# haesungpyun/seoul_tourism_recommendation_NGCF

Measured on AMD Instinct MI355X. Metric: NGCF 3-layer forward: propagated edges/sec + achieved HBM GB/s, d=128, higher is better.
Workload: dtype f32

## Files before the change

seoul_tourism_recommendation_ngcf_amd/csrc/common.h:

```cpp
#ifndef NGCF_COMMON_H
#define NGCF_COMMON_H

#include <hip/hip_runtime.h>

#include <algorithm>
#include <cstdarg>
#include <cstdint>
#include <cstdio>
#include <cstdlib>
#include <cstring>
#include <numeric>
#include <thread>
#include <vector>

#include "../../include/ngcf_hip.h"

inline thread_local char g_err[512] = "";

inline int fail(int code, const char *fmt, ...)
{
    va_list ap;
    va_start(ap, fmt);
    vsnprintf(g_err, sizeof(g_err), fmt, ap);
    va_end(ap);
    return code;
}

#define HIP_TRY(expr)                                                                          \
    do {                                                                                       \
        hipError_t e_ = (expr);                                                                \
        if (e_ != hipSuccess)                                                                  \
            return fail(NGCF_ERR_HIP, "%s failed: %s (%s:%d)", #expr, hipGetErrorString(e_),   \
                        __FILE__, __LINE__);                                                   \
    } while (0)

#define LAUNCH_CHECK()                                                                         \
    do {                                                                                       \
        hipError_t e_ = hipGetLastError();                                                     \
        if (e_ != hipSuccess)                                                                  \
            return fail(NGCF_ERR_HIP, "kernel launch failed: %s (%s:%d)", hipGetErrorString(e_), \
                        __FILE__, __LINE__);                                                   \
    } while (0)


struct NgcfOptions {
    int no_fork = 0;
    int no_slicing = 0;
    int no_ldstab = 0;
    int no_panel_split = 0;
    int no_tail_table = 0;
    int no_pad_product = 0;
    int64_t fork_min = 200000000;
    int dense_direct = 1;
    int dense_resident = 4;
    int dense_resident_min_rows = 106496;
    int dense_small_tiles = 1;
    int dense_tall = 1;
    int t_rows_bitmap = 1;
    int bwd_input_resident = 1;
    int select_no_lds = 0;
    int slice_max_mb = 48;
    int swept_lpe = 16;
    int swept_cut = 4;
    int swept_no_moments = 0;
    int swept_order_rows = 0;
    int swept_debug = 0;
    int swept_window_kb = 0;
    int swept_spin = 500;
    int swept_lead = -2;
    int swept_sync_every = 1;
    int swept_prio_kb = 256;
    int swept_prio_graded = 1;
};
extern NgcfOptions g_opts;
const NgcfOptions &ngcf_opts();


constexpr int kMaxDevices = 64;
inline int current_device_slot()
{
    int dev = 0;
    if (hipGetDevice(&dev) != hipSuccess || dev < 0) dev = 0;
    return dev % kMaxDevices;
}

template <auto kernel> static hipError_t allow_full_lds(int bytes = 160 * 1024)
{
    static bool set[kMaxDevices] = {};
    const int dev_i = current_device_slot();
    if (set[dev_i]) return hipSuccess;
    const hipError_t e = hipFuncSetAttribute(reinterpret_cast<const void *>(kernel), hipFuncAttributeMaxDynamicSharedMemorySize, bytes);
    set[dev_i] = e == hipSuccess;
    return e;
}

inline int64_t align_up(int64_t x, int64_t a) { return (x + a - 1) / a * a; }
inline bool aligned16(const void *p) { return (reinterpret_cast<uintptr_t>(p) & 15) == 0; }


inline int grid_for(int64_t n, int block)

{
    int64_t g = (n + block - 1) / block;
    if (g < 1) g = 1;
    if (g > 256 * 16) g = 256 * 16;
    return (int)g;
}



struct ngcf_csr {
    int64_t n_rows = 0, n_cols = 0, nnz = 0;
    int64_t max_row_len = 0;
    int64_t *rowptr = nullptr;
    int32_t *colidx = nullptr;
    float *vals = nullptr;
    bool owns = false;
    int64_t cap = 0, pos_len = 0;
    int32_t *pos = nullptr;
    int32_t *scan_blk = nullptr;
    bool borrows_plan = false;
    const struct ngcf_csr *filter_src = nullptr;
    int32_t seg_len = 0;
    int64_t n_seg = 0, n_heavy = 0;
    int32_t *seg_row = nullptr;
    int64_t *seg_begin = nullptr;
    int32_t *heavy_row = nullptr;
    int64_t *heavy_seg_ptr = nullptr;
    struct RowGroup {
        int64_t begin, end;
        bool sliceable;
        int32_t col_lo, col_hi;
        bool lds_table = false;
    };
    std::vector<RowGroup> groups;
    int mode = 0;
    struct SegSet {
        int64_t n_seg = 0, n_heavy = 0;
        int32_t *seg_row = nullptr;
        int64_t *seg_begin = nullptr;
        int32_t *heavy_row = nullptr;
        int64_t *heavy_seg_ptr = nullptr;
    };
    struct Swept {
        struct Part {
            int64_t row_lo = 0, row_hi = 0;
            int waves = 0, rows_per_wave = 0;
            int lpe = 16;
            int32_t n_rowpass = 0, n_win = 0, win_cols = 0, col_lo = 0, col_hi = 0;
            int64_t n_slots = 0, n_partial = 0, n_heavy = 0, partial_base = 0;
            int64_t *tptr = nullptr;
            int32_t *e_pack = nullptr;
            float *e_val = nullptr;
            int32_t *dst = nullptr;
            int32_t *prow = nullptr;
            int32_t *heavy_row = nullptr;
            int64_t *heavy_seg_ptr = nullptr;
        };
        std::vector<Part> parts;
        std::vector<char> group_swept;
        SegSet out;
        int64_t n_partial = 0;
        uint32_t *barrier = nullptr;
        mutable hipStream_t barrier_owner[4] = {nullptr, nullptr, nullptr, nullptr};
        mutable int barrier_used = 0;
        int built_mode = 0;
        int lpe = 16;
    } swept;
};


static const int32_t kLdsTableRows = 512;
static const int32_t kDefaultSegLen = 2048;
static inline int32_t default_seg_len(int64_t nnz)
{
    int32_t s = 64;
    while (s < kDefaultSegLen && (int64_t)s * 4096 < nnz) s *= 2;
    return s;
}

void free_swept(ngcf_csr *c);
int build_swept_plan(ngcf_csr *c, hipStream_t stream);
bool swept_usable(const ngcf_csr *c, int64_t ldE, int d);
void prof_mark(hipStream_t stream, int which);

__host__ __device__ inline uint64_t fmix64(uint64_t x)
{
    x ^= x >> 33;
    x *= 0xff51afd7ed558ccdULL;
    x ^= x >> 33;
    x *= 0xc4ceb9fe1a85ec53ULL;
    x ^= x >> 33;
    return x;
}
__device__ inline uint32_t mix32(uint64_t x) { return (uint32_t)fmix64(x); }

__device__ __forceinline__ uint32_t msg_drop_thr(float drop_p)
{
    return drop_p > 0.f ? (uint32_t)((double)drop_p * 4294967296.0) : 0u;
}
__device__ __forceinline__ float msg_drop(float v, uint64_t seed, int64_t row, int col, uint32_t thr, float keep_scale)
{
    const uint32_t h = mix32(seed ^ ((uint64_t)row * 0x9E3779B97F4A7C15ULL + (uint64_t)col));
    return h < thr ? 0.f : v * keep_scale;
}

constexpr uint64_t kSeedPtrTag = 0xD5EDull;
__device__ inline uint64_t resolve_seed(uint64_t s)
{
    if ((s >> 48) == kSeedPtrTag) s = *reinterpret_cast<const uint64_t *>(s & 0xFFFFFFFFFFFFull);
    const uint32_t lo = __builtin_amdgcn_readfirstlane((uint32_t)s), hi = __builtin_amdgcn_readfirstlane((uint32_t)(s >> 32));
    return ((uint64_t)hi << 32) | lo;
}

struct EdgeDrop {
    int n;
    uint32_t thr;
    uint64_t seed[4];
    int transposed;
};

struct EdgeDropR {
    int n;
    uint32_t thr;
    uint64_t s0, s1, s2, s3;
// ... 116 lines not shown
```

seoul_tourism_recommendation_ngcf_amd/csrc/csr.hip:

```cpp
#include "common.h"

extern "C" const char *ngcf_last_error(void) { return g_err; }
extern "C" const char *ngcf_target_arch(void) { return "gfx950"; }
extern "C" int ngcf_version(void) { return NGCF_ABI_VERSION; }

NgcfOptions g_opts;

namespace {
struct OptField {
    const char *name;
    int NgcfOptions::*i;
    int64_t NgcfOptions::*l;
};
const OptField kOptFields[] = {
    {"no_fork", &NgcfOptions::no_fork, nullptr},
    {"no_slicing", &NgcfOptions::no_slicing, nullptr},
    {"no_ldstab", &NgcfOptions::no_ldstab, nullptr},
    {"no_panel_split", &NgcfOptions::no_panel_split, nullptr},
    {"no_tail_table", &NgcfOptions::no_tail_table, nullptr},
    {"no_pad_product", &NgcfOptions::no_pad_product, nullptr},
    {"fork_min", nullptr, &NgcfOptions::fork_min},
    {"dense_direct", &NgcfOptions::dense_direct, nullptr},
    {"dense_resident", &NgcfOptions::dense_resident, nullptr},
    {"dense_resident_min_rows", &NgcfOptions::dense_resident_min_rows, nullptr},
    {"dense_small_tiles", &NgcfOptions::dense_small_tiles, nullptr},
    {"dense_tall", &NgcfOptions::dense_tall, nullptr},
    {"bwd_input_resident", &NgcfOptions::bwd_input_resident, nullptr},
    {"t_rows_bitmap", &NgcfOptions::t_rows_bitmap, nullptr},
    {"select_no_lds", &NgcfOptions::select_no_lds, nullptr},
    {"slice_max_mb", &NgcfOptions::slice_max_mb, nullptr},
    {"swept_lpe", &NgcfOptions::swept_lpe, nullptr},
    {"swept_cut", &NgcfOptions::swept_cut, nullptr},
    {"swept_no_moments", &NgcfOptions::swept_no_moments, nullptr},
    {"swept_order_rows", &NgcfOptions::swept_order_rows, nullptr},
    {"swept_debug", &NgcfOptions::swept_debug, nullptr},
    {"swept_window_kb", &NgcfOptions::swept_window_kb, nullptr},
    {"swept_spin", &NgcfOptions::swept_spin, nullptr},
    {"swept_lead", &NgcfOptions::swept_lead, nullptr},
    {"swept_sync_every", &NgcfOptions::swept_sync_every, nullptr},
    {"swept_prio_kb", &NgcfOptions::swept_prio_kb, nullptr},
    {"swept_prio_graded", &NgcfOptions::swept_prio_graded, nullptr},
};
bool g_opts_read = false;
}

extern "C" int ngcf_options_from_env(void)
{
    NgcfOptions o;
    for (const OptField &f : kOptFields) {
        char var[64] = "NGCF_";
        size_t n = strlen(var);
        for (const char *p = f.name; *p && n + 1 < sizeof(var); ++p) var[n++] = (char)((*p >= 'a' && *p <= 'z') ? *p - 32 : *p);
        var[n] = 0;
        const char *e = getenv(var);
        if (!e) continue;
        const long long v = *e ? atoll(e) : 1;
        if (f.i) o.*(f.i) = (int)(*e && (*e == '-' || (*e >= '0' && *e <= '9')) ? v : 1);
        else o.*(f.l) = v;
    }
    if (const char *e = getenv("NGCF_SWEPT_ORDER")) o.swept_order_rows = !strcmp(e, "rows");
    g_opts = o;
    g_opts_read = true;
    return NGCF_OK;
}

const NgcfOptions &ngcf_opts()
{
    if (!g_opts_read) ngcf_options_from_env();
    return g_opts;
}

extern "C" int ngcf_set_option(const char *name, int64_t value)
{
    if (!name) return fail(NGCF_ERR_ARG, "ngcf_set_option: null name");
    (void)ngcf_opts();
    for (const OptField &f : kOptFields)
        if (!strcmp(f.name, name)) {
            if (f.i) g_opts.*(f.i) = (int)value;
            else g_opts.*(f.l) = value;
            return NGCF_OK;
        }
    return fail(NGCF_ERR_ARG, "ngcf_set_option: unknown option '%s'", name);
}


static void free_plan(ngcf_csr *c)
{
    if (c->borrows_plan) {
        c->seg_row = nullptr;
        c->heavy_row = nullptr;
        c->heavy_seg_ptr = nullptr;
        c->borrows_plan = false;
    }
    if (c->seg_row) (void)hipFree(c->seg_row);
    if (c->seg_begin) (void)hipFree(c->seg_begin);
    if (c->heavy_row) (void)hipFree(c->heavy_row);
    if (c->heavy_seg_ptr) (void)hipFree(c->heavy_seg_ptr);
    c->seg_row = nullptr;
    c->seg_begin = nullptr;
    c->heavy_row = nullptr;
    c->heavy_seg_ptr = nullptr;
    c->n_seg = c->n_heavy = 0;
}

extern "C" void ngcf_csr_free(ngcf_csr_t *c)
{
    if (!c) return;
    free_plan(c);
    free_swept(c);
    if (c->owns) {
        if (c->rowptr) (void)hipFree(c->rowptr);
        if (c->colidx) (void)hipFree(c->colidx);
        if (c->vals) (void)hipFree(c->vals);
    }
    if (c->pos) (void)hipFree(c->pos);
    if (c->scan_blk) (void)hipFree(c->scan_blk);
    delete c;
}

extern "C" int64_t ngcf_csr_nnz(const ngcf_csr_t *c) { return c ? c->nnz : -1; }
extern "C" int64_t ngcf_csr_n_rows(const ngcf_csr_t *c) { return c ? c->n_rows : -1; }
extern "C" int64_t ngcf_csr_n_cols(const ngcf_csr_t *c) { return c ? c->n_cols : -1; }
extern "C" int64_t ngcf_csr_n_segments(const ngcf_csr_t *c) { return c ? c->n_seg : -1; }
extern "C" int64_t ngcf_csr_max_row_len(const ngcf_csr_t *c) { return c ? c->max_row_len : -1; }
extern "C" int64_t ngcf_csr_swept_rows(const ngcf_csr_t *c)
{
    if (!c) return -1;
    int64_t n = 0;
    for (const auto &p : c->swept.parts) n += p.row_hi - p.row_lo;
    return n;
}
extern "C" const int64_t *ngcf_csr_rowptr(const ngcf_csr_t *c) { return c ? c->rowptr : nullptr; }
extern "C" const int32_t *ngcf_csr_colidx(const ngcf_csr_t *c) { return c ? c->colidx : nullptr; }
extern "C" const float *ngcf_csr_vals(const ngcf_csr_t *c) { return c ? c->vals : nullptr; }

__global__ void coo_check_kernel(const int64_t *__restrict__ rows, const int64_t *__restrict__ cols,
                                 int64_t nnz, int64_t n_rows, int64_t n_cols, int32_t *flags)
{
    int64_t i = (int64_t)blockIdx.x * blockDim.x + threadIdx.x;
    const int64_t stride = (int64_t)gridDim.x * blockDim.x;
    bool unsorted = false, bad = false;
    for (; i < nnz; i += stride) {
        const int64_t r = rows[i], c = cols[i];
        bad |= (r < 0) | (r >= n_rows) | (c < 0) | (c >= n_cols);
        if (i + 1 < nnz) unsorted |= rows[i + 1] < r;
    }
    if (unsorted) atomicOr(&flags[0], 1);
    if (bad) atomicOr(&flags[1], 1);
}

__global__ void coo_rowptr_kernel(const int64_t *__restrict__ rows, int64_t nnz, int64_t n_rows,
                                  int64_t *__restrict__ rowptr)
{
    const int64_t r = (int64_t)blockIdx.x * blockDim.x + threadIdx.x;
    if (r > n_rows) return;
    int64_t lo = 0, hi = nnz;
    while (lo < hi) {
        const int64_t mid = (lo + hi) >> 1;
        if (rows[mid] < r)
            lo = mid + 1;
        else
            hi = mid;
    }
    rowptr[r] = lo;
}

__global__ void coo_copy_kernel(const int64_t *__restrict__ cols, const float *__restrict__ vals, int64_t nnz,
                                int32_t *__restrict__ colidx, float *__restrict__ out_vals)
{
    int64_t i = (int64_t)blockIdx.x * blockDim.x + threadIdx.x;
    const int64_t stride = (int64_t)gridDim.x * blockDim.x;
    for (; i < nnz; i += stride) {
        colidx[i] = (int32_t)cols[i];
        out_vals[i] = vals[i];
    }
}


__global__ void row_colrange_kernel(const int64_t *__restrict__ rowptr, const int32_t *__restrict__ colidx,
                                    int64_t n_rows, int group_rows, int32_t *__restrict__ blk_min, int32_t *__restrict__ blk_max)
{
    const int64_t row = (int64_t)blockIdx.x * blockDim.x + threadIdx.x;
    if (row >= n_rows) return;
    int32_t lo = INT32_MAX, hi = -1;
    for (int64_t e = rowptr[row]; e < rowptr[row + 1]; ++e) {
        const int32_t c = colidx[e];
        lo = c < lo ? c : lo;
        hi = c > hi ? c : hi;
    }
    if (hi >= 0) {
        atomicMin(&blk_min[row / group_rows], lo);
        atomicMax(&blk_max[row / group_rows], hi);
    }
}
// ... 451 lines not shown
```

seoul_tourism_recommendation_ngcf_amd/csrc/spmm_swept.hip:

```cpp
#include "spmm_device.h"

namespace {
constexpr int kLdsBytes = 36 * 16 * 256;
constexpr int kSweptWGs = 256;
constexpr int kRing = 8;
constexpr int kRowBits = 24;
constexpr int kColMask = (1 << kRowBits) - 1;

template <typename F>
void parallel_for(int64_t n, F &&fn, int64_t min_parallel = 64)
{
    unsigned nt = std::thread::hardware_concurrency();
    if (nt > 16) nt = 16;
    if (nt < 1) nt = 1;
    if ((int64_t)nt > n) nt = (unsigned)std::max<int64_t>(n, 1);
    if (n < min_parallel || nt == 1) {
        fn(0, n);
        return;
    }
    std::vector<std::thread> th;
    const int64_t chunk = (n + nt - 1) / nt;
    for (unsigned t = 0; t < nt; ++t) {
        const int64_t lo = t * chunk, hi = std::min<int64_t>(n, lo + chunk);
        if (lo >= hi) break;
        th.emplace_back([&fn, lo, hi]() { fn(lo, hi); });
    }
    for (auto &t : th) t.join();
}

void free_part(ngcf_csr::Swept::Part &p)
{
    if (p.tptr) (void)hipFree(p.tptr);
    if (p.e_pack) (void)hipFree(p.e_pack);
    if (p.e_val) (void)hipFree(p.e_val);
    if (p.dst) (void)hipFree(p.dst);
    if (p.prow) (void)hipFree(p.prow);
    if (p.heavy_row) (void)hipFree(p.heavy_row);
    if (p.heavy_seg_ptr) (void)hipFree(p.heavy_seg_ptr);
    p = ngcf_csr::Swept::Part();
}

void free_segset(ngcf_csr::SegSet &s)
{
    if (s.seg_row) (void)hipFree(s.seg_row);
    if (s.seg_begin) (void)hipFree(s.seg_begin);
    if (s.heavy_row) (void)hipFree(s.heavy_row);
    if (s.heavy_seg_ptr) (void)hipFree(s.heavy_seg_ptr);
    s = ngcf_csr::SegSet();
}

template <typename T>
int upload(T **dptr, const std::vector<T> &h, hipStream_t stream)
{
    HIP_TRY(hipMalloc(dptr, sizeof(T) * std::max<size_t>(h.size(), 1)));
    if (!h.empty()) HIP_TRY(hipMemcpyAsync(*dptr, h.data(), sizeof(T) * h.size(), hipMemcpyHostToDevice, stream));
    return NGCF_OK;
}

struct Piece {
    int64_t row;
    int64_t begin, end, count;
    int32_t off, step;
    int64_t src;
};

int build_part(const ngcf_csr *c, const ngcf_csr::RowGroup &grp, bool force, hipStream_t stream, ngcf_csr::Swept::Part &part, int LPE)
{
    const int kSW = LPE * 4, kEPR = 64 / LPE, kLdsRows = kLdsBytes / (kSW * 4);
    const int64_t row_lo = grp.begin, row_hi = grp.end, n = row_hi - row_lo;
    const int32_t col_lo = grp.col_lo, col_hi = grp.col_hi;
    if (n <= 0 || col_hi < col_lo) return NGCF_OK;
    if (col_hi > kColMask) return NGCF_OK;
    std::vector<int64_t> rp((size_t)n + 1);
    HIP_TRY(hipMemcpyAsync(rp.data(), c->rowptr + row_lo, sizeof(int64_t) * rp.size(), hipMemcpyDeviceToHost, stream));
    HIP_TRY(hipStreamSynchronize(stream));
    const int64_t e0 = rp[0], nnz = rp[(size_t)n] - e0;
    if (nnz <= 0) return NGCF_OK;
    if (!force && nnz < ((int64_t)1 << 22)) return NGCF_OK;
    const int64_t cap = (int64_t)kSweptWGs * kLdsRows;
    const int waves = 16;
    const int RW = kLdsRows / waves;
    const int64_t n_wave_slots = (int64_t)kSweptWGs * waves;
    if (!force) {
        const double span = (double)col_hi - col_lo + 1;
        const double reuse = (double)nnz / span * std::min(1.0, (double)(cap / 8) / (double)n);
        if (reuse < 3.0 || span * kSW * 4 < (double)(8 << 20)) return NGCF_OK;
    }
    std::vector<int32_t> col((size_t)nnz);
    std::vector<float> val((size_t)nnz);
    HIP_TRY(hipMemcpyAsync(col.data(), c->colidx + e0, sizeof(int32_t) * (size_t)nnz, hipMemcpyDeviceToHost, stream));
    HIP_TRY(hipMemcpyAsync(val.data(), c->vals + e0, sizeof(float) * (size_t)nnz, hipMemcpyDeviceToHost, stream));
    HIP_TRY(hipStreamSynchronize(stream));
    for (auto &x : rp) x -= e0;
    int64_t n_rowpass = std::max<int64_t>(1, (n + cap - 1) / cap), n_tasks = 0, T = 0, n_partial = 0;
    std::vector<Piece> pieces;
    std::vector<int32_t> heavy_row;
    std::vector<int64_t> heavy_ptr;
    for (;; ++n_rowpass) {
        n_tasks = n_rowpass * n_wave_slots;
        T = std::max<int64_t>(64, (nnz + n_tasks - 1) / n_tasks);
        const int64_t Tp = std::max<int64_t>(64, T / std::max(2, ngcf_opts().swept_cut));
        pieces.clear();
        heavy_row.clear();
        heavy_ptr.assign(1, 0);
        n_partial = 0;
        for (int64_t r = 0; r < n; ++r) {
            const int64_t b = rp[(size_t)r], e = rp[(size_t)r + 1], len = e - b;
            if (len <= Tp) {
                pieces.push_back({r, b, e, len, 0, 1, r});
            } else {
                const int64_t k = (len + Tp - 1) / Tp;
                heavy_row.push_back((int32_t)(row_lo + r));
                for (int64_t j = 0; j < k; ++j) pieces.push_back({-1 - n_partial++, b, e, (len - j + k - 1) / k, (int32_t)j, (int32_t)k, r});
                heavy_ptr.push_back(n_partial);
            }
        }
        if ((int64_t)pieces.size() <= n_tasks * RW) break;
        if (n_rowpass > (int64_t)1 << 20) return fail(NGCF_ERR_ARG, "swept plan: cannot place %zu pieces", pieces.size());
    }
    if (n_tasks * RW >= (int64_t)1 << 31 || n_partial >= ((int64_t)1 << 31) - 2) return fail(NGCF_ERR_ARG, "swept plan: matrix too large");
    constexpr int kDealK = 8, kDealBucket = 256;
    const bool balance_moments = !ngcf_opts().swept_no_moments;
    std::vector<float> mom;
    if (balance_moments) {
        const int64_t span = (int64_t)col_hi - col_lo + 1;
        std::vector<int64_t> ccnt((size_t)span + 1, 0);
        for (int64_t x = 0; x < nnz; ++x) ccnt[(size_t)(col[(size_t)x] - col_lo) + 1]++;
        for (int64_t c = 0; c < span; ++c) ccnt[(size_t)c + 1] += ccnt[(size_t)c];
        std::vector<float> ctab((size_t)span * kDealK);
        parallel_for(span, [&](int64_t lo, int64_t hi) {
            for (int64_t c = lo; c < hi; ++c) {
                const double xpos = (0.5 * (double)(ccnt[(size_t)c] + ccnt[(size_t)c + 1])) / (double)nnz;
                for (int k = 0; k < kDealK; ++k) ctab[(size_t)c * kDealK + k] = (float)cos((k + 1) * 3.14159265358979323846 * xpos);
            }
        });
        mom.assign(pieces.size() * kDealK, 0.f);
        parallel_for((int64_t)pieces.size(), [&](int64_t lo, int64_t hi) {
            for (int64_t pi = lo; pi < hi; ++pi) {
                const Piece &pc = pieces[(size_t)pi];
                float acc[kDealK] = {0};
                for (int64_t x = pc.begin + pc.off; x < pc.end; x += pc.step) {
                    const float *t = &ctab[(size_t)(col[(size_t)x] - col_lo) * kDealK];
                    for (int k = 0; k < kDealK; ++k) acc[k] += t[k];
                }
                for (int k = 0; k < kDealK; ++k) mom[(size_t)pi * kDealK + k] = acc[k];
            }
        });
    }
    std::vector<int64_t> order(pieces.size());
    std::iota(order.begin(), order.end(), 0);
    std::stable_sort(order.begin(), order.end(), [&](int64_t a, int64_t b) { return pieces[(size_t)a].count > pieces[(size_t)b].count; });
    std::vector<int64_t> load((size_t)n_tasks, 0), by_load((size_t)n_tasks);
    std::vector<float> tmom(balance_moments ? (size_t)n_tasks * kDealK : 0, 0.f);
    std::vector<int64_t> task_piece((size_t)(n_tasks * RW), -1);
    for (int64_t lvl = 0; lvl * n_tasks < (int64_t)pieces.size(); ++lvl) {
        std::iota(by_load.begin(), by_load.end(), 0);
        std::stable_sort(by_load.begin(), by_load.end(), [&](int64_t a, int64_t b) { return load[(size_t)a] < load[(size_t)b]; });
        const int64_t lo = lvl * n_tasks, hi = std::min<int64_t>((int64_t)pieces.size(), lo + n_tasks);
// ... 151 lines not shown
            bucket_hist(t, hist);
            for (int64_t w = 0; w < n_win; ++w) {
                rounds[(size_t)w] = (tptr[(size_t)(t * n_win + w) + 1] - tptr[(size_t)(t * n_win + w)]) / kEPR;
                int32_t run = 0;
                for (int lr = 0; lr < RW; ++lr) {
                    const int32_t cnt = hist[(size_t)w * RW + lr];
                    hist[(size_t)w * RW + lr] = run;
                    run += cnt;
                }
            }
            for (int lr = 0; lr < RW; ++lr) {
                const int64_t pi = task_piece[(size_t)(t * RW + lr)];
                if (pi < 0) continue;
                const Piece &pc = pieces[(size_t)pi];
                for (int64_t x = pc.begin + pc.off; x < pc.end; x += pc.step) {
                    const int64_t w = (col[(size_t)x] - col_lo) / win_cols;
                    const int64_t k = hist[(size_t)w * RW + lr]++, R = rounds[(size_t)w];
                    const int64_t pos = tptr[(size_t)(t * n_win + w)] + (k % R) * kEPR + k / R;
                    e_pack[(size_t)pos] = (int32_t)((uint32_t)lr << kRowBits) | col[(size_t)x];
                    e_val[(size_t)pos] = val[(size_t)x];
                }
            }
            for (int64_t w = 0; w < n_win; ++w) {
                const int64_t b0 = tptr[(size_t)(t * n_win + w)], b1 = tptr[(size_t)(t * n_win + w) + 1];
                if (b0 == b1) continue;
                const int32_t spare = (int32_t)((uint32_t)RW << kRowBits) | (e_pack[(size_t)b0] & kColMask);
                for (int64_t x = b0; x < b1; ++x)
                    if (e_pack[(size_t)x] < 0) e_pack[(size_t)x] = spare;
            }
        }
    });
    std::vector<int32_t> dst((size_t)(n_tasks * RW), -1), prow((size_t)(n_tasks * RW), 0);
    for (size_t i = 0; i < dst.size(); ++i) {
        if (task_piece[i] < 0) continue;
        const int64_t r = pieces[(size_t)task_piece[i]].row;
        dst[i] = r >= 0 ? (int32_t)(row_lo + r) : (int32_t)(-2 - (-1 - r));
        prow[i] = (int32_t)(row_lo + pieces[(size_t)task_piece[i]].src);
    }
    if (ngcf_opts().swept_debug) {
        int64_t mx = 0, mn = INT64_MAX;
        for (int64_t t = 0; t < n_tasks; ++t) {
            const int64_t s = tptr[(size_t)((t + 1) * n_win)] - tptr[(size_t)(t * n_win)];
            mx = std::max(mx, s);
            mn = std::min(mn, s);
        }
        fprintf(stderr, "[swept plan] rows [%lld, %lld) nnz %lld cols [%d, %d]: %d waves x %d rows, %lld row passes, %lld windows x %d "
                        "cols, T %lld, pieces %zu (partial %lld), slots %lld (+%.1f%%), per task %lld..%lld\n",
                (long long)row_lo, (long long)row_hi, (long long)nnz, col_lo, col_hi, waves, RW, (long long)n_rowpass, (long long)n_win,
                win_cols, (long long)T, pieces.size(), (long long)n_partial, (long long)n_slots,
                100.0 * (double)(n_slots - nnz) / (double)nnz, (long long)mn, (long long)mx);
    }
    part.row_lo = row_lo;
    part.row_hi = row_hi;
    part.rows_per_wave = RW;
    part.lpe = LPE;
    part.n_rowpass = (int32_t)n_rowpass;
    part.n_win = (int32_t)n_win;
    part.win_cols = win_cols;
    part.col_lo = col_lo;
    part.col_hi = col_hi;
    part.n_slots = n_slots;
    part.n_partial = n_partial;
    part.n_heavy = (int64_t)heavy_row.size();
    int rc = upload(&part.tptr, tptr, stream);
    if (rc == NGCF_OK) rc = upload(&part.e_pack, e_pack, stream);
    if (rc == NGCF_OK) rc = upload(&part.e_val, e_val, stream);
    if (rc == NGCF_OK) rc = upload(&part.dst, dst, stream);
    if (rc == NGCF_OK) rc = upload(&part.prow, prow, stream);
    if (rc == NGCF_OK && part.n_heavy > 0) rc = upload(&part.heavy_row, heavy_row, stream);
    if (rc == NGCF_OK && part.n_heavy > 0) rc = upload(&part.heavy_seg_ptr, heavy_ptr, stream);
    if (rc == NGCF_OK && hipStreamSynchronize(stream) != hipSuccess) rc = fail(NGCF_ERR_HIP, "swept plan: upload failed");
    if (rc != NGCF_OK) {
        free_part(part);
        return rc;
    }
    part.waves = waves;
    return NGCF_OK;
}
}

void free_swept(ngcf_csr *c)
{
    ngcf_csr::Swept &w = c->swept;
    for (auto &p : w.parts) free_part(p);
    free_segset(w.out);
    if (w.barrier) (void)hipFree(w.barrier);
    w = ngcf_csr::Swept();
}

int build_swept_plan(ngcf_csr *c, hipStream_t stream)
{
    free_swept(c);
    ngcf_csr::Swept &w = c->swept;
    w.built_mode = c->mode;
    w.lpe = ngcf_opts().swept_lpe == 32 ? 32 : 16;
    if (c->mode < 2 || c->n_rows == 0 || c->nnz == 0) return NGCF_OK;
    int dev = 0, cus = 0;
    if (hipGetDevice(&dev) != hipSuccess || hipDeviceGetAttribute(&cus, hipDeviceAttributeMultiprocessorCount, dev) != hipSuccess ||
        cus != kSweptWGs) {
        static bool warned = false;
        if (!warned) {
            warned = true;
            fprintf(stderr, "[ngcf] note: this device reports %d CUs, not %d (an MI355X in SPX mode): the L2-swept SpMM plan is not built and the "
                            "products run on the row-wise kernels (about half the speed on large graphs); ngcf_csr_swept_rows() returns 0\n",
                    cus, kSweptWGs);
        }
        return NGCF_OK;
    }
    w.group_swept.assign(c->groups.size(), 0);
    for (size_t g = 0; g < c->groups.size(); ++g) {
        ngcf_csr::Swept::Part p;
        const int rc = build_part(c, c->groups[g], c->mode == 2, stream, p, w.lpe);
        if (rc != NGCF_OK) {
            free_swept(c);
            return rc;
        }
        if (p.waves == 0) continue;
        w.group_swept[g] = 1;
        w.parts.push_back(p);
    }
    if (w.parts.empty()) return NGCF_OK;
    std::vector<int64_t> rp((size_t)c->n_rows + 1);
    HIP_TRY(hipMemcpyAsync(rp.data(), c->rowptr, sizeof(int64_t) * rp.size(), hipMemcpyDeviceToHost, stream));
    HIP_TRY(hipStreamSynchronize(stream));
    std::vector<int32_t> seg_row, heavy_row;
    std::vector<int64_t> seg_begin, heavy_ptr(1, 0);
    for (size_t g = 0; g < c->groups.size(); ++g) {
        if (w.group_swept[g]) continue;
        for (int64_t r = c->groups[g].begin; r < c->groups[g].end; ++r) {
            if (rp[(size_t)r + 1] - rp[(size_t)r] <= c->seg_len) continue;
            heavy_row.push_back((int32_t)r);
            for (int64_t b = rp[(size_t)r]; b < rp[(size_t)r + 1]; b += c->seg_len) {
                seg_row.push_back((int32_t)r);
                seg_begin.push_back(b);
            }
            heavy_ptr.push_back((int64_t)seg_row.size());
        }
    }
    w.out.n_seg = (int64_t)seg_row.size();
    w.out.n_heavy = (int64_t)heavy_row.size();
    int64_t base = w.out.n_seg;
    for (auto &p : w.parts) {
        p.partial_base = base;
        base += p.n_partial;
        w.n_partial += p.n_partial;
    }
    int rc = NGCF_OK;
    if (w.out.n_seg > 0) {
        rc = upload(&w.out.seg_row, seg_row, stream);
        if (rc == NGCF_OK) rc = upload(&w.out.seg_begin, seg_begin, stream);
        if (rc == NGCF_OK) rc = upload(&w.out.heavy_row, heavy_row, stream);
        if (rc == NGCF_OK) rc = upload(&w.out.heavy_seg_ptr, heavy_ptr, stream);
    }
    if (rc == NGCF_OK && (hipMalloc(&w.barrier, sizeof(uint32_t) * 32 * 8 * 4) != hipSuccess || hipStreamSynchronize(stream) != hipSuccess))
        rc = fail(NGCF_ERR_HIP, "swept plan: allocation failed");
    if (rc != NGCF_OK) free_swept(c);
    return rc;
}

bool swept_usable(const ngcf_csr *c, int64_t ldE, int d)
{
    const ngcf_csr::Swept &w = c->swept;
    if (w.parts.empty() || c->mode < 2 || d % (w.lpe * 4) != 0) return false;
    for (const auto &p : w.parts)
        if (((int64_t)p.col_hi + 1) * ldE * 4 > (int64_t)UINT32_MAX) return false;
    return true;
}

typedef float f32x4 __attribute__((ext_vector_type(4)));
#ifndef NGCF_SWEPT_LABW
#define NGCF_SWEPT_LABW 2
#endif

constexpr int kMaxLaunchParts = 4;
struct SweptPartArgs {
    const int64_t *tptr;
    const int32_t *e_pack;
    const float *e_val;
    const int32_t *dst;
    const int32_t *prow;
    float *partial;
    int n_rowpass, n_win, lead;
};
struct SweptLaunch {
    SweptPartArgs part[kMaxLaunchParts];
    int n_parts;
};

template <int LPE, int RW, int NW, bool DROP>
__global__ __launch_bounds__(NW * 64) void spmm_swept_kernel(SweptLaunch L, int n_slices, const float *__restrict__ E,
                                                             int64_t ldE, float *__restrict__ out, int64_t ldo, int dp, unsigned *bar,
                                                             int max_spin, int sync_k, unsigned prio_cols, int prio_graded,
                                                             EdgeDrop dr_in)
{
    const EdgeDropR dr = resolve_drop(dr_in);
    constexpr int kSW = LPE * 4, kEPR = 64 / LPE, kCH = 16 * kEPR;
    __shared__ float acc_lds[NW * (RW + 1) * kSW];
    __shared__ unsigned wg_cnt[kRing];
    __shared__ int perm_lds;
    __shared__ unsigned xcc_id;
    __shared__ unsigned wg_front;
    const int wave = threadIdx.x >> 6, lane = threadIdx.x & 63;
    const int g = lane / LPE, p = lane % LPE;
    const int held = (lane & 15) * kEPR + g;
    float *wacc = acc_lds + wave * ((RW + 1) * kSW);
    if (threadIdx.x < kRing) wg_cnt[threadIdx.x] = 0;
    if (threadIdx.x == 0) {
        xcc_id = __builtin_amdgcn_s_getreg((3 << 11) | 20) & 7u;
        perm_lds = L.part[0].lead;
        wg_front = 0;
    }
    __syncthreads();
    unsigned *ctr = bar + xcc_id * 32;
    const unsigned members = gridDim.x / 8;
    int perm = L.part[0].lead;
    int step0 = 0;
    const unsigned ld_bytes = (unsigned)ldE * 4u;
    int sweep_no = 0;
    for (int pi = 0; pi < L.n_parts; ++pi) {
    const int64_t *__restrict__ tptr = L.part[pi].tptr;
    const int32_t *__restrict__ e_pack = L.part[pi].e_pack;
    const float *__restrict__ e_val = L.part[pi].e_val;
    const int32_t *__restrict__ dst = L.part[pi].dst;
    float *__restrict__ partial = L.part[pi].partial;
    const int n_rowpass = L.part[pi].n_rowpass, n_win = L.part[pi].n_win, lead = L.part[pi].lead;
    const bool sync = lead >= 0;
    for (int rp = 0; rp < n_rowpass; ++rp) {
        const int64_t task = ((int64_t)rp * gridDim.x + blockIdx.x) * NW + wave;
        const int64_t *tp = tptr + task * n_win;
        const int64_t beg = tp[0], end = tp[n_win];
        int my_row = 0, my_row_hi = 0;
        if (DROP && lane < RW) my_row = L.part[pi].prow[task * RW + lane];
        if (DROP && RW > 64 && lane + 64 < RW) my_row_hi = L.part[pi].prow[task * RW + 64 + lane];
        for (int slice = 0; slice < n_slices; ++slice, ++sweep_no, step0 += (n_win + sync_k - 1) / sync_k) {
            const char *Eb = reinterpret_cast<const char *>(E + slice * kSW);
            for (int i = lane; i < (RW + 1) * kSW; i += 64) wacc[i] = 0.f;
            int b = 0;
            int64_t wend = tp[1], wend_next = n_win > 1 ? tp[2] : end;
            auto arrive = [&](int s) {
                if (sync && lane == 0) {
                    const unsigned old = atomicAdd(&wg_cnt[s % kRing], 1u);
                    if ((old + 1) % NW == 0)
                        __hip_atomic_fetch_add(ctr + (s % kRing), 1u, __ATOMIC_RELAXED, __HIP_MEMORY_SCOPE_AGENT);
                }
            };
            auto cross = [&](int64_t pos, bool crossed) {
                while (b < n_win - 1 && pos >= wend) {
                    if ((b + 1) % sync_k == 0) arrive(step0 + b / sync_k);
                    ++b;
                    wend = wend_next;
                    wend_next = b + 2 <= n_win ? tp[b + 2] : end;
                    crossed = true;
                }
                const int s = step0 + b / sync_k;
                if (crossed && sync && max_spin > 0 && perm < s) {
                    perm = __hip_atomic_load(&perm_lds, __ATOMIC_RELAXED, __HIP_MEMORY_SCOPE_WORKGROUP);
                    int spins = 0;
                    while (perm < s) {
                        const unsigned mine = lane < kRing ? __hip_atomic_load(ctr + lane, __ATOMIC_RELAXED, __HIP_MEMORY_SCOPE_AGENT) : 0u;
                        int t = perm - lead;
                        for (int k = 0; k < kRing - 2 - lead; ++k, ++t) {
                            const unsigned have = __builtin_amdgcn_readlane(mine, t % kRing);
                            if (have < members * (unsigned)(t / kRing + 1)) break;
                        }
                        perm = t + lead;
                        if (perm >= s) break;
                        if (++spins >= max_spin) {
                            max_spin = 0;
                            break;
                        }
                        __builtin_amdgcn_s_sleep(2);
                    }
                    if (lane == 0) atomicMax(&perm_lds, perm);
                }
            };
            const int idle_pk = end > beg ? (RW << kRowBits) | (e_pack[beg] & kColMask) : 0;
            auto load_entries = [&](int64_t pos, int &pk, float &v) {
                const int64_t idx = pos + held;
                const int64_t idc = idx < end ? idx : end - 1;
                const int pk_l = e_pack[idc];
                const float v_l = e_val[idc];
                pk = idx < end ? pk_l : idle_pk;
                v = idx < end ? v_l : 0.f;
                if (DROP) {
                    const int lr = (pk >> kRowBits) & 0x7f;
                    int grow = __shfl(my_row, lr < RW ? lr & 63 : 0);
                    if (RW > 64) {
                        const int hi = __shfl(my_row_hi, lr & 63);
                        grow = lr >= 64 && lr < RW ? hi : grow;
                    }
                    v = edge_keep(dr, grow, pk & kColMask) ? v : 0.f;
                }
            };
            if (end > beg) {
                int pkA, pkB;
                float vA, vB;
                f32x4 xa[8], xb[8];
                unsigned offA;
                const unsigned lane_off = p * 16;
#define NGCF_GATHER(buf, u, j) buf[j] = *reinterpret_cast<const f32x4 *>(Eb + ((unsigned)row_bcast<u>((int)offA) + lane_off));
#define NGCF_GATHER_LO(x) NGCF_GATHER(x, 0, 0) NGCF_GATHER(x, 1, 1) NGCF_GATHER(x, 2, 2) NGCF_GATHER(x, 3, 3) NGCF_GATHER(x, 4, 4) NGCF_GATHER(x, 5, 5) NGCF_GATHER(x, 6, 6) NGCF_GATHER(x, 7, 7)
#define NGCF_GATHER_HI(x) NGCF_GATHER(x, 8, 0) NGCF_GATHER(x, 9, 1) NGCF_GATHER(x, 10, 2) NGCF_GATHER(x, 11, 3) NGCF_GATHER(x, 12, 4) NGCF_GATHER(x, 13, 5) NGCF_GATHER(x, 14, 6) NGCF_GATHER(x, 15, 7)
#define NGCF_ACC(buf, u, j)                                                                        \
    {                                                                                             \
        const int pku = row_bcast<u>(pkA);                                                        \
        const float vu = row_bcast<u>(vA);                                                        \
        if (pku >= 0) {                                                                           \
            f32x4 *a = reinterpret_cast<f32x4 *>(wacc + (pku >> kRowBits) * kSW + p * 4);         \
            f32x4 t = *a;                                                                         \
            t.x = fmaf(vu, buf[j].x, t.x);                                                          \
            t.y = fmaf(vu, buf[j].y, t.y);                                                          \
            t.z = fmaf(vu, buf[j].z, t.z);                                                          \
            t.w = fmaf(vu, buf[j].w, t.w);                                                          \
            *a = t;                                                                               \
        }                                                                                         \
    }
#define NGCF_ACC_LO(x) NGCF_ACC(x, 0, 0) NGCF_ACC(x, 1, 1) NGCF_ACC(x, 2, 2) NGCF_ACC(x, 3, 3) NGCF_ACC(x, 4, 4) NGCF_ACC(x, 5, 5) NGCF_ACC(x, 6, 6) NGCF_ACC(x, 7, 7)
#define NGCF_ACC_HI(x) NGCF_ACC(x, 8, 0) NGCF_ACC(x, 9, 1) NGCF_ACC(x, 10, 2) NGCF_ACC(x, 11, 3) NGCF_ACC(x, 12, 4) NGCF_ACC(x, 13, 5) NGCF_ACC(x, 14, 6) NGCF_ACC(x, 15, 7)
                load_entries(beg, pkA, vA);
                cross(beg, true);
                offA = (unsigned)(pkA & kColMask) * ld_bytes;
                NGCF_GATHER_LO(xa)
                const unsigned sweep_tag = (unsigned)(sweep_no & 0xff) << kRowBits;
                for (int64_t pos = beg; pos < end; pos += kCH) {
                    if (prio_cols) {
                        const unsigned mine = sweep_tag | (unsigned)(__builtin_amdgcn_readfirstlane(pkA) & kColMask);
                        unsigned front = 0;
                        if (lane == 0) front = atomicMax(&wg_front, mine);
                        front = (unsigned)__builtin_amdgcn_readfirstlane((int)front);
                        const unsigned lag = front > mine ? front - mine : 0u;
                        if (prio_graded) {
                            if (lag > 4 * prio_cols) __builtin_amdgcn_s_setprio(3);
                            else if (lag > 2 * prio_cols) __builtin_amdgcn_s_setprio(2);
                            else if (lag > prio_cols) __builtin_amdgcn_s_setprio(1);
                            else __builtin_amdgcn_s_setprio(0);
                        } else {
                            if (lag > prio_cols) __builtin_amdgcn_s_setprio(3);
                            else __builtin_amdgcn_s_setprio(0);
                        }
                    }
                    load_entries(pos + kCH, pkB, vB);
                    if (pos + 8 * kEPR < end) cross(pos + 8 * kEPR, false);
                    NGCF_GATHER_HI(xb)
                    __builtin_amdgcn_s_waitcnt(0xF70 | (NGCF_SWEPT_LABW & 0xf));
                    NGCF_ACC_LO(xa)
                    if (pos + kCH < end) cross(pos + kCH, false);
                    offA = (unsigned)(pkB & kColMask) * ld_bytes;
                    NGCF_GATHER_LO(xa)
                    __builtin_amdgcn_s_waitcnt(0xF70 | (NGCF_SWEPT_LABW & 0xf));
                    NGCF_ACC_HI(xb)
                    pkA = pkB;
                    vA = vB;
                }
#undef NGCF_GATHER
#undef NGCF_GATHER_LO
#undef NGCF_GATHER_HI
#undef NGCF_ACC
#undef NGCF_ACC_LO
#undef NGCF_ACC_HI
            }
            cross(INT64_MAX - 1, false);
            arrive(step0 + (n_win - 1) / sync_k);
            for (int r0 = 0; r0 < RW; r0 += kEPR) {
                const int r = r0 + g;
                if (r < RW) {
                    const int drow = dst[task * RW + r];
                    if (drow != -1) {
                        float *o = drow >= 0 ? out + (int64_t)drow * ldo : partial + (int64_t)(-2 - drow) * dp;
                        *reinterpret_cast<f32x4 *>(o + slice * kSW + p * 4) = *reinterpret_cast<const f32x4 *>(wacc + r * kSW + p * 4);
                    }
                }
            }
        }
    }
    }
}

int launch_swept(const ngcf_csr *c, const float *E, int64_t ldE, int d, float *out, int64_t ldo, float *partial, int dp,
                 hipStream_t stream, const EdgeDrop &dr)
{
    const ngcf_csr::Swept &w = c->swept;
    const NgcfOptions &o = ngcf_opts();
    const int max_spin = o.swept_spin;
    const int lead_env = o.swept_lead;
    const int sync_k = std::max(1, o.swept_sync_every);
    const int kSW = w.lpe * 4;
    const unsigned prio_cols = (unsigned)std::max(0, o.swept_prio_kb) * 1024u / (kSW * 4);
    const int prio_graded = o.swept_prio_graded;
    for (const auto &p : w.parts) {
        SweptLaunch L{};
        const int lead = std::min(lead_env != -2 ? lead_env : (p.n_win >= 8 ? 2 : 1), kRing - 4);
        L.part[L.n_parts++] = SweptPartArgs{p.tptr, p.e_pack, p.e_val, p.dst, p.prow, partial ? partial + p.partial_base * (int64_t)dp : nullptr,
                                            p.n_rowpass, p.n_win, lead};
        int bi = 0;
        for (; bi < w.barrier_used && w.barrier_owner[bi] != stream; ++bi) {}
        if (bi == w.barrier_used) {
            if (w.barrier_used < 4) w.barrier_owner[w.barrier_used++] = stream;
            else bi = 3;
        }
        unsigned *bar_blk = w.barrier + (size_t)bi * 32 * 8;
        HIP_TRY(hipMemsetAsync(bar_blk, 0, sizeof(uint32_t) * 32 * 8, stream));
#define NGCF_SWEPT_LAUNCH(LPE_, RW_, NW_, DROP_)                                                                                    \
    spmm_swept_kernel<LPE_, RW_, NW_, DROP_><<<dim3(kSweptWGs), NW_ * 64, 0, stream>>>(L, d / kSW, E, ldE, out, ldo, dp, bar_blk, \
                                                                                max_spin, sync_k, prio_cols, prio_graded, dr)
        if (w.lpe == 32 && dr.n > 0) NGCF_SWEPT_LAUNCH(32, 18, 16, true);
        else if (w.lpe == 32) NGCF_SWEPT_LAUNCH(32, 18, 16, false);
        else if (dr.n > 0) NGCF_SWEPT_LAUNCH(16, 36, 16, true);
        else NGCF_SWEPT_LAUNCH(16, 36, 16, false);
#undef NGCF_SWEPT_LAUNCH
        LAUNCH_CHECK();
    }
    for (const auto &p : w.parts) {
        if (p.n_heavy == 0) continue;
        spmm_fixup_kernel<4><<<dim3((unsigned)((p.n_heavy + 3) / 4)), 256, 0, stream>>>(
            p.heavy_row, p.heavy_seg_ptr, p.n_heavy, partial + p.partial_base * (int64_t)dp, dp, d, out, ldo);
        LAUNCH_CHECK();
    }
    return NGCF_OK;
}
```

Baseline: 28.44 billion.

## Add per-XCD workgroup lead brake board and self-resetting swept barrier

Result: no change. 28.34 billion (-0.4%).

```diff
diff --git a/seoul_tourism_recommendation_ngcf_amd/csrc/common.h b/seoul_tourism_recommendation_ngcf_amd/csrc/common.h
--- a/seoul_tourism_recommendation_ngcf_amd/csrc/common.h
+++ b/seoul_tourism_recommendation_ngcf_amd/csrc/common.h
@@ -71,6 +71,9 @@
     int swept_sync_every = 1;
     int swept_prio_kb = 256;
     int swept_prio_graded = 1;
+    int swept_wg_lead_kb = 0;
+    int swept_wg_step_kb = 256;
+    int swept_part_order = 0;
 };
 extern NgcfOptions g_opts;
 const NgcfOptions &ngcf_opts();
diff --git a/seoul_tourism_recommendation_ngcf_amd/csrc/csr.hip b/seoul_tourism_recommendation_ngcf_amd/csrc/csr.hip
--- a/seoul_tourism_recommendation_ngcf_amd/csrc/csr.hip
+++ b/seoul_tourism_recommendation_ngcf_amd/csrc/csr.hip
@@ -40,6 +40,9 @@
     {"swept_sync_every", &NgcfOptions::swept_sync_every, nullptr},
     {"swept_prio_kb", &NgcfOptions::swept_prio_kb, nullptr},
     {"swept_prio_graded", &NgcfOptions::swept_prio_graded, nullptr},
+    {"swept_wg_lead_kb", &NgcfOptions::swept_wg_lead_kb, nullptr},
+    {"swept_wg_step_kb", &NgcfOptions::swept_wg_step_kb, nullptr},
+    {"swept_part_order", &NgcfOptions::swept_part_order, nullptr},
 };
 bool g_opts_read = false;
 }
diff --git a/seoul_tourism_recommendation_ngcf_amd/csrc/spmm_swept.hip b/seoul_tourism_recommendation_ngcf_amd/csrc/spmm_swept.hip
--- a/seoul_tourism_recommendation_ngcf_amd/csrc/spmm_swept.hip
+++ b/seoul_tourism_recommendation_ngcf_amd/csrc/spmm_swept.hip
@@ -4,6 +4,7 @@
 constexpr int kLdsBytes = 36 * 16 * 256;
 constexpr int kSweptWGs = 256;
 constexpr int kRing = 8;
+constexpr int kBoardOff = 8 * 32, kDoneOff = 2 * 8 * 32, kBlockWords = kDoneOff + 32;
 constexpr int kRowBits = 24;
 constexpr int kColMask = (1 << kRowBits) - 1;
 
@@ -461,7 +462,9 @@
         if (rc == NGCF_OK) rc = upload(&w.out.heavy_row, heavy_row, stream);
         if (rc == NGCF_OK) rc = upload(&w.out.heavy_seg_ptr, heavy_ptr, stream);
     }
-    if (rc == NGCF_OK && (hipMalloc(&w.barrier, sizeof(uint32_t) * 32 * 8 * 4) != hipSuccess || hipStreamSynchronize(stream) != hipSuccess))
+    if (rc == NGCF_OK && (hipMalloc(&w.barrier, sizeof(uint32_t) * kBlockWords * 4) != hipSuccess ||
+                          hipMemsetAsync(w.barrier, 0, sizeof(uint32_t) * kBlockWords * 4, stream) != hipSuccess ||
+                          hipStreamSynchronize(stream) != hipSuccess))
         rc = fail(NGCF_ERR_HIP, "swept plan: allocation failed");
     if (rc != NGCF_OK) free_swept(c);
     return rc;
@@ -496,19 +499,23 @@
     int n_parts;
 };
 
-template <int LPE, int RW, int NW, bool DROP>
+template <int LPE, int RW, int NW, bool DROP, bool BOARD>
 __global__ __launch_bounds__(NW * 64) void spmm_swept_kernel(SweptLaunch L, int n_slices, const float *__restrict__ E,
                                                              int64_t ldE, float *__restrict__ out, int64_t ldo, int dp, unsigned *bar,
                                                              int max_spin, int sync_k, unsigned prio_cols, int prio_graded,
-                                                             EdgeDrop dr_in)
+                                                             unsigned brake_cols_in, int pub_shift, EdgeDrop dr_in)
 {
     const EdgeDropR dr = resolve_drop(dr_in);
+    const unsigned brake_cols = BOARD ? brake_cols_in : 0u;
     constexpr int kSW = LPE * 4, kEPR = 64 / LPE, kCH = 16 * kEPR;
     __shared__ float acc_lds[NW * (RW + 1) * kSW];
     __shared__ unsigned wg_cnt[kRing];
     __shared__ int perm_lds;
     __shared__ unsigned xcc_id;
     __shared__ unsigned wg_front;
+    __shared__ unsigned xcd_min;
+    __shared__ unsigned board_slot;
+    __shared__ unsigned wg_last;
     const int wave = threadIdx.x >> 6, lane = threadIdx.x & 63;
     const int g = lane / LPE, p = lane % LPE;
     const int held = (lane & 15) * kEPR + g;
@@ -518,9 +525,20 @@
         xcc_id = __builtin_amdgcn_s_getreg((3 << 11) | 20) & 7u;
         perm_lds = L.part[0].lead;
         wg_front = 0;
+        xcd_min = 0;
+        board_slot = 0;
+        if (brake_cols) board_slot = __hip_atomic_fetch_add(bar + xcc_id * 32 + kRing, 1u, __ATOMIC_RELAXED, __HIP_MEMORY_SCOPE_AGENT) & 31u;
     }
     __syncthreads();
     unsigned *ctr = bar + xcc_id * 32;
+    unsigned *board = bar + kBoardOff + xcc_id * 32;
+    int max_brake = max_spin;
+    auto board_min = [&](unsigned mine) {
+        unsigned v = lane < 32 ? __hip_atomic_load(board + lane, __ATOMIC_RELAXED, __HIP_MEMORY_SCOPE_AGENT) : ~0u;
+        if ((v ^ mine) >> kRowBits) v = ~0u;
+        for (int o = 16; o > 0; o >>= 1) v = min(v, (unsigned)__shfl_xor((int)v, o));
+        return (unsigned)__builtin_amdgcn_readfirstlane((int)v);
+    };
     const unsigned members = gridDim.x / 8;
     int perm = L.part[0].lead;
     int step0 = 0;
@@ -632,13 +650,14 @@
                 NGCF_GATHER_LO(xa)
                 const unsigned sweep_tag = (unsigned)(sweep_no & 0xff) << kRowBits;
                 for (int64_t pos = beg; pos < end; pos += kCH) {
-                    if (prio_cols) {
+                    if (prio_cols | brake_cols) {
                         const unsigned mine = sweep_tag | (unsigned)(__builtin_amdgcn_readfirstlane(pkA) & kColMask);
                         unsigned front = 0;
                         if (lane == 0) front = atomicMax(&wg_front, mine);
                         front = (unsigned)__builtin_amdgcn_readfirstlane((int)front);
                         const unsigned lag = front > mine ? front - mine : 0u;
-                        if (prio_graded) {
+                        if (!prio_cols) {
+                        } else if (prio_graded) {
                             if (lag > 4 * prio_cols) __builtin_amdgcn_s_setprio(3);
                             else if (lag > 2 * prio_cols) __builtin_amdgcn_s_setprio(2);
                             else if (lag > prio_cols) __builtin_amdgcn_s_setprio(1);
@@ -646,6 +665,25 @@
                         } else {
                             if (lag > prio_cols) __builtin_amdgcn_s_setprio(3);
                             else __builtin_amdgcn_s_setprio(0);
+                        }
+                        if (brake_cols) {
+                            const bool publish = mine > front && ((mine ^ front) >> pub_shift) != 0;
+                            unsigned least = __hip_atomic_load(&xcd_min, __ATOMIC_RELAXED, __HIP_MEMORY_SCOPE_WORKGROUP);
+                            least = (unsigned)__builtin_amdgcn_readfirstlane((int)least);
+                            auto ahead = [&]() { return ((least ^ mine) >> kRowBits) == 0 && mine > least && mine - least > brake_cols; };
+                            if (publish || (max_brake > 0 && ahead())) {
+                                if (publish && lane == 0) __hip_atomic_store(board + board_slot, mine, __ATOMIC_RELAXED, __HIP_MEMORY_SCOPE_AGENT);
+                                least = board_min(mine);
+                                for (int spins = 0; max_brake > 0 && ahead();) {
+                                    if (++spins >= max_brake) {
+                                        max_brake = 0;
+                                        break;
+                                    }
+                                    __builtin_amdgcn_s_sleep(2);
+                                    least = board_min(mine);
+                                }
+                                if (lane == 0) __hip_atomic_store(&xcd_min, least, __ATOMIC_RELAXED, __HIP_MEMORY_SCOPE_WORKGROUP);
+                            }
                         }
                     }
                     load_entries(pos + kCH, pkB, vB);
@@ -683,6 +721,16 @@
         }
     }
     }
+    if (brake_cols && lane == 0) __hip_atomic_store(board + board_slot, ~0u, __ATOMIC_RELAXED, __HIP_MEMORY_SCOPE_AGENT);
+    asm volatile("s_waitcnt vmcnt(0)" ::: "memory");
+    __syncthreads();
+    if (threadIdx.x == 0) {
+        const unsigned done = __hip_atomic_fetch_add(bar + kDoneOff, 1u, __ATOMIC_RELAXED, __HIP_MEMORY_SCOPE_AGENT) + 1u;
+        wg_last = done % gridDim.x == 0;
+    }
+    __syncthreads();
+    if (wg_last)
+        for (int i = threadIdx.x; i < kDoneOff; i += NW * 64) __hip_atomic_store(bar + i, 0u, __ATOMIC_RELAXED, __HIP_MEMORY_SCOPE_AGENT);
 }
 
 int launch_swept(const ngcf_csr *c, const float *E, int64_t ldE, int d, float *out, int64_t ldo, float *partial, int dp,
@@ -696,7 +744,13 @@
     const int kSW = w.lpe * 4;
     const unsigned prio_cols = (unsigned)std::max(0, o.swept_prio_kb) * 1024u / (kSW * 4);
     const int prio_graded = o.swept_prio_graded;
-    for (const auto &p : w.parts) {
+    const int pub_cols = std::max(1, o.swept_wg_step_kb) * 1024 / (kSW * 4);
+    int pub_shift = 0;
+    while ((2 << pub_shift) <= pub_cols) ++pub_shift;
+    const unsigned brake_cols = o.swept_wg_lead_kb > 0 ? (unsigned)std::min<int64_t>((int64_t)o.swept_wg_lead_kb * 1024 / (kSW * 4), kColMask) + (1u << pub_shift) : 0u;
+    const size_t n_parts = w.parts.size();
+    for (size_t pi = 0; pi < n_parts; ++pi) {
+        const auto &p = w.parts[o.swept_part_order ? n_parts - 1 - pi : pi];
         SweptLaunch L{};
         const int lead = std::min(lead_env != -2 ? lead_env : (p.n_win >= 8 ? 2 : 1), kRing - 4);
         L.part[L.n_parts++] = SweptPartArgs{p.tptr, p.e_pack, p.e_val, p.dst, p.prow, partial ? partial + p.partial_base * (int64_t)dp : nullptr,
@@ -707,16 +761,21 @@
             if (w.barrier_used < 4) w.barrier_owner[w.barrier_used++] = stream;
             else bi = 3;
         }
-        unsigned *bar_blk = w.barrier + (size_t)bi * 32 * 8;
-        HIP_TRY(hipMemsetAsync(bar_blk, 0, sizeof(uint32_t) * 32 * 8, stream));
-#define NGCF_SWEPT_LAUNCH(LPE_, RW_, NW_, DROP_)                                                                                    \
-    spmm_swept_kernel<LPE_, RW_, NW_, DROP_><<<dim3(kSweptWGs), NW_ * 64, 0, stream>>>(L, d / kSW, E, ldE, out, ldo, dp, bar_blk, \
-                                                                                max_spin, sync_k, prio_cols, prio_graded, dr)
+        unsigned *bar_blk = w.barrier + (size_t)bi * kBlockWords;
+#define NGCF_SWEPT_LAUNCH_B(LPE_, RW_, NW_, DROP_, BOARD_)                                                                                  \
+    spmm_swept_kernel<LPE_, RW_, NW_, DROP_, BOARD_><<<dim3(kSweptWGs), NW_ * 64, 0, stream>>>(L, d / kSW, E, ldE, out, ldo, dp, bar_blk, \
+                                                                                max_spin, sync_k, prio_cols, prio_graded, brake_cols, pub_shift, dr)
+#define NGCF_SWEPT_LAUNCH(LPE_, RW_, NW_, DROP_)                          \
+    do {                                                                  \
+        if (brake_cols) NGCF_SWEPT_LAUNCH_B(LPE_, RW_, NW_, DROP_, true); \
+        else NGCF_SWEPT_LAUNCH_B(LPE_, RW_, NW_, DROP_, false);           \
+    } while (0)
         if (w.lpe == 32 && dr.n > 0) NGCF_SWEPT_LAUNCH(32, 18, 16, true);
         else if (w.lpe == 32) NGCF_SWEPT_LAUNCH(32, 18, 16, false);
         else if (dr.n > 0) NGCF_SWEPT_LAUNCH(16, 36, 16, true);
         else NGCF_SWEPT_LAUNCH(16, 36, 16, false);
 #undef NGCF_SWEPT_LAUNCH
+#undef NGCF_SWEPT_LAUNCH_B
         LAUNCH_CHECK();
     }
     for (const auto &p : w.parts) {
```
